# swapUniba/Deep_CBRS_Amar_Renaissance

Hardware: AMD Instinct MI355X
Metric: (user,item) pairs scored/sec, ML-1M basic-gnn 2-layer, 1/2/4/8 MI355X (higher is better)
Workload: dtype f32; 1 GPU; ml1m(s=64) user-item graph: N=590592 nodes, nnz(A_hat)=55909934, 12089292 test pairs; econfigs/basic-gnn.yaml grid1 BasicGCN d=8 L=2 concat, dense [24,24], clf [48,48]; one propagation + per-entity towers + all pairs (shuffled order) per step (hoisted); scale=64, parallelism=single GPU (step replayed from a hipGraph)

## Files before the change

deep_cbrs_amar_renaissance_amd/capi.py:

```python
import ctypes
import os

import torch

_HERE = os.path.dirname(os.path.abspath(__file__))
LIB_PATH = os.path.join(_HERE, 'libamar_hip.so')

ACT_NONE, ACT_RELU, ACT_SIGMOID = 0, 1, 2
ACT_CODES = {None: ACT_NONE, 'linear': ACT_NONE, 'relu': ACT_RELU, 'sigmoid': ACT_SIGMOID}
AGG_SUM, AGG_MAX, AGG_MIN = 0, 1, 2
AGG_CODES = {'sum': AGG_SUM, 'max': AGG_MAX, 'min': AGG_MIN}
SPMM_BIAS, SPMM_RELU, SPMM_ACCUM, SPMM_ACCUM_DIV, SPMM_SCALE_NEXT, SPMM_SAGE_TAIL, SPMM_LT_NOPAIRS = 1, 2, 4, 8, 16, 32, 64

_P = ctypes.c_void_p
_I32, _I64, _U32, _F32 = ctypes.c_int32, ctypes.c_int64, ctypes.c_uint32, ctypes.c_float

SIGNATURES = {
    'amar_version': (ctypes.c_int, []),
    'amar_error_string': (ctypes.c_char_p, [ctypes.c_int]),
    'amar_last_hip_error': (ctypes.c_int, []),
    'amar_spmm_csr_f32': (ctypes.c_int, [_P, _P, _P, _P, _I64, _P, _I64, _I32, _I32, _U32, _P,
                                         _P, _I64, _P, _I64, _F32, _P]),
    'amar_spmm_sj_f32': (ctypes.c_int, [_P, _P, _P, _I32, _P, _I64, _P, _I64, _I32, _I32, _U32, _P,
                                        _P, _I64, _P, _I64, _F32, _P, _I32, _P, _I64, _P]),
# ... 4 lines not shown
    'amar_gat_lt_rows_per_wave': (ctypes.c_int, [_I32]),
    'amar_colmax_f32': (ctypes.c_int, [_P, _I64, _P, _P]),
    'amar_spmm_lt_f32': (ctypes.c_int, [_P, _P, _P, _P, _P, _P, _P, _I32, _I32, _I32, _P, _P, _P, _I64, _I32, _P, _P, _I64, _I32, _I32, _U32, _P,
                                        _P, _I64, _P, _I64, _F32, _P, _I32, _P, _I64, _P]),
    'amar_propagate_route': (ctypes.c_int, [_I32, _I64, _I64, _I32, _U32, _P]),
    'amar_gat_xs_f32': (ctypes.c_int, [_P, _P, _I32, _P, _I64, _I32, _P, _P, _P, _P, _P, _P, _I64, _I32, _I32, _I32, _I32, _P]),
    'amar_gcn_layer_f32': (ctypes.c_int, [_P, _P, _P, _P, _I64, _I32, _P, _P, _I64, _P, _I32, _P, _I64, _I32, _P]),
    'amar_rowwise_xw_f32': (ctypes.c_int, [_P, _I64, _I32, _P, _I32, _P, _I64, _P, _I64, _P, _P, _P, _P, _P, _I32, _P]),
    'amar_rowwise_xw_gather_f32': (ctypes.c_int, [_P, _I64, _I32, _P, _P, _I32, _P, _I64, _P, _I32, _P]),
    'amar_sage_layer_f32': (ctypes.c_int, [_P, _P, _P, _I64, _I32, _P, _P, _I32, _P, _I64, _I32, _I32, _P]),
    'amar_sage_tail_f32': (ctypes.c_int, [_P, _I64, _P, _I64, _I32, _P, _P, _I32, _P, _I64, _I64, _P]),
    'amar_sage_layer_agg_f32': (ctypes.c_int, [_P, _P, _P, _I64, _I32, _P, _P, _I32, _P, _I64, _I32, _I32, _I32, _P]),
    'amar_sage_aggregate_f32': (ctypes.c_int, [_P, _P, _P, _I64, _I32, _P, _I64, _P, _I64, _I32, _I32, _I32, _P]),
    'amar_sage_aggregate_bwd_f32': (ctypes.c_int, [_P, _P, _P, _I64, _P, _I64, _P, _I64, _P, _I64, _I32, _P, _P, _I64, _I32, _I32, _P]),
    'amar_gat_layer_f32': (ctypes.c_int, [_P, _P, _P, _I64, _I32, _P, _P, _P, _P, _I64, _I32, _I32, _P]),
    'amar_rowwise_xw_heads_f32': (ctypes.c_int, [_P, _I64, _I32, _P, _I32, _I32, _P, _I64, _P, _P, _P, _I32, _P]),
    'amar_gat_heads_f32': (ctypes.c_int, [_P, _P, _P, _I64, _I32, _I32, _P, _P, _P, _I64, _P, _I32, _I32, _I32, _P]),
    'amar_dense_f32': (ctypes.c_int, [_P, _I64, _P, _P, _P, _P, _I64, _I64, _I32, _I32, _I32, _P]),
    'amar_dense_route': (ctypes.c_int, [_P, _I64, _P, _P, _P, _P, _I64, _I64, _I32, _I32, _I32, _P]),
    'amar_dense_split_bytes': (ctypes.c_int64, [_I32, _I32]),
    'amar_dense_split_pack_f32': (ctypes.c_int, [_P, _I32, _I32, _P]),
    'amar_dense_split_f32': (ctypes.c_int, [_P, _I64, _P, _P, _P, _P, _I64, _I64, _I32, _I32, _I32, _P]),
    'amar_chain_pack_floats': (ctypes.c_int64, [_P, _I32]),
    'amar_chain_pack_f32': (ctypes.c_int, [_P, _P, _P, _I32, _P]),
    'amar_chain_f32': (ctypes.c_int, [_P, _I64, _I32, _P, _I32, _P, _I64, _I32, _P, _I32, _I32, _I32, _P, _P, _P, _I32, _P, _I64, _I64, _P]),
    'amar_chain_indexed_f32': (ctypes.c_int, [_P, _I64, _I32, _P, _I32, _P, _I64, _I32, _P, _I32, _I32, _I32, _P, _P, _P, _I32, _P, _I64, _P, _I64, _P]),
    'amar_chain_segments_f32': (ctypes.c_int, [_P, _P, _P, _I32, _P, _I32, _P, _P, _P, _I32, _P, _I64, _I64, _P]),
    'amar_chain_route': (ctypes.c_int, [_P, _I64, _I32, _P, _I32, _P, _I64, _I32, _P, _I32, _I32, _I32, _P, _P, _P, _I32, _P, _I64, _P, _I64, _P]),
    'amar_chain_segments_route': (ctypes.c_int, [_P, _P, _P, _I32, _P, _I32, _P, _P, _P, _I32, _P, _I64, _I64, _P]),
    'amar_dual_chain_f32': (ctypes.c_int, [_P, _P, _P, _P, _P, _P, _P, _P, _I32, _I32, _I32, _P, _P, _P, _I32, _P, _P, _I64, _I64, _P]),
    'amar_dual_chain_indexed_f32': (ctypes.c_int, [_P, _P, _P, _P, _P, _P, _P, _P, _I32, _I32, _I32, _P, _P, _P, _I32, _P, _P, _I64, _P, _I64, _P]),
    'amar_copy_columns_f32': (ctypes.c_int, [_P, _I64, _P, _I32, _P, _I64, _I64, _I32, _P]),
    'amar_scatter_f32': (ctypes.c_int, [_P, _P, _P, _I64, _I64, _P, _I32, _P]),
    'amar_reduce_layers_f32': (ctypes.c_int, [_P, _I64, _I32, _I32, _P, _I64, _I64, _I32, _P]),
    'amar_reduce_layers_wsum_f32': (ctypes.c_int, [_P, _I64, _I32, _I32, _P, _P, _I64, _I64, _P]),
    'amar_reduce_layers_wsum_bwd_scratch': (ctypes.c_int64, []),
    'amar_reduce_layers_wsum_bwd_f32': (ctypes.c_int, [_P, _I64, _I32, _I32, _P, _P, _I64, _P, _I64, _P, _P, _I64, _P]),
    'amar_act_bwd_f32': (ctypes.c_int, [_P, _I64, _P, _I64, _P, _I64, _I64, _I32, _I32, _P]),
    'amar_wgrad_scratch_floats': (ctypes.c_int64, [_I64, _I32, _I32]),
    'amar_wgrad_f32': (ctypes.c_int, [_P, _I64, _P, _I64, _I64, _I32, _I32, _P, _P, _P, _P]),
    'amar_dense_stack_f32': (ctypes.c_int, [_P, _I64, _P, _P, _I64, _I32, _P, _P, _P, _P, _P, _P, _I64, _P]),
    'amar_dense_stack_pair_f32': (ctypes.c_int, [_P, _P, _P]),
    'amar_dense_stack_route': (ctypes.c_int, [_P, _I64, _P, _P, _I64, _I32, _P, _P, _P, _P, _P, _P, _I64, _P]),
    'amar_dense_stack_bwd_groups': (ctypes.c_int64, [_I64]),
    'amar_dense_stack_bwd_workspace_floats': (ctypes.c_int64, [_I64, _I32, _P]),
    'amar_dense_stack_bwd_pair_f32': (ctypes.c_int, [_P, _P, _P]),
    'amar_dense_stack_bwd_f32': (ctypes.c_int, [_P, _I64, _P, _I64, _I32, _P, _P, _P, _P, _P, _P, _I64, _P, _P, _P, _I32, _I64, _P]),
    'amar_dense_stack_bwd_route': (ctypes.c_int, [_P, _I64, _P, _I64, _I32, _P, _P, _P, _P, _P, _P, _I64, _P, _P, _P, _I32, _I64, _P]),
    'amar_dense_bwd_workspace_floats': (ctypes.c_int64, [_I64, _I32, _I32]),
    'amar_dense_bwd_groups': (ctypes.c_int64, [_I64]),
    'amar_dense_bwd_f32': (ctypes.c_int, [_P, _I64, _P, _I64, _P, _I64, _P, _I32, _P, _I64, _P, _P, _P, _I64, _P, _I64, _I32, _I32, _P]),
    'amar_dense_bwd_route': (ctypes.c_int, [_P, _I64, _P, _I64, _P, _I64, _P, _I32, _P, _I64, _P, _P, _P, _I64, _I64, _I32, _I32, _P]),
    'amar_bce_grad_f32': (ctypes.c_int, [_P, _I64, _P, _P, _P, _I64, _P]),
    'amar_wgrad_route': (ctypes.c_int, [_P, _I64, _P, _I64, _I64, _I32, _I32, _P, _P, _P]),
    'amar_scatter_add_rows_route': (ctypes.c_int, [_I64, _I32, _P]),
    'amar_scatter_add_rows_f32': (ctypes.c_int, [_P, _I64, _P, _I32, _P, _I64, _I64, _I32, _P]),
    'amar_add_inplace_f32': (ctypes.c_int, [_P, _I64, _P, _I64, _I64, _I32, _F32, _P]),
    'amar_row_affine_f32': (ctypes.c_int, [_P, _I64, _P, _I64, _P, _P, _I64, _I64, _I32, _P]),
    'amar_l2norm_fwd_f32': (ctypes.c_int, [_P, _I64, _P, _I64, _P, _P, _I64, _I64, _I32, _I32, _P]),
    'amar_l2norm_bwd_f32': (ctypes.c_int, [_P, _I64, _P, _I64, _P, _P, _I64, _I64, _I32, _I32, _P]),
    'amar_gat_bwd_f32': (ctypes.c_int, [_P, _P, _P, _I64, _I32, _P, _P, _P, _I64, _P, _I64, _P, _P, _P, _P, _P, _P, _P, _P, _I64,
                                        _I32, _I32, _P]),
    'amar_gat_bwd_directed_f32': (ctypes.c_int, [_P, _P, _P, _P, _P, _I64, _I32, _P, _P, _P, _I64, _P, _I64, _P, _P, _P, _P, _P, _P, _P, _P, _I64,
                                                 _I32, _I32, _P]),
    'amar_gat_heads_bwd_f32': (ctypes.c_int, [_P, _P, _P, _P, _P, _I64, _I32, _I32, _P, _P, _I64, _P, _I64, _P, _P, _P, _P, _P, _P, _P, _P, _I64,
                                              _I32, _I32, _I32, _P]),
# ... 797 lines not shown


def dual_chain_supported(D, n_branch_dims_equal, trunk_dims):
    return (D % 16 == 0 and D <= 64 and n_branch_dims_equal and len(trunk_dims) >= 3 and trunk_dims[0] == 2 * D
            and trunk_dims[-1] == 1 and len(set(trunk_dims[1:-1])) == 1 and trunk_dims[1] <= 64 and trunk_dims[1] % 4 == 0)


def dual_chain(tables_a, tables_b, ids_a, ids_b, bases_a, bases_b, D, in_act, branch_acts, trunk_dims, trunk_acts, wpack, out,
               out_index=None):
    P = out.shape[0]
    arr = lambda vals, ctype: (ctype * 2)(*vals)
    A = arr([_ptr(t, torch.float32, 'A') for t in tables_a], ctypes.c_void_p)
    B = arr([_ptr(t, torch.float32, 'B') for t in tables_b], ctypes.c_void_p)
    IA = arr([_ptr(t, torch.int32, 'ida') for t in ids_a], ctypes.c_void_p)
    IB = arr([_ptr(t, torch.int32, 'idb') for t in ids_b], ctypes.c_void_p)
    for ids in list(ids_a) + list(ids_b):
        if ids is not None and ids.numel() != P:
            raise ValueError("dual_chain: one id per output row expected")
    lda = arr([_ld(t, 'A') for t in tables_a], ctypes.c_int64)
    ldb = arr([_ld(t, 'B') for t in tables_b], ctypes.c_int64)
    ba, bb = arr([int(b) for b in bases_a], ctypes.c_int32), arr([int(b) for b in bases_b], ctypes.c_int32)
    bacts = (ctypes.c_int32 * max(1, len(branch_acts)))(*[ACT_CODES[a] for a in branch_acts])
    tdims = (ctypes.c_int32 * len(trunk_dims))(*trunk_dims)
    tacts = (ctypes.c_int32 * len(trunk_acts))(*[ACT_CODES[a] for a in trunk_acts])
    if out_index is not None and out_index.numel() != P:
        raise ValueError("dual_chain: out_index must have one entry per output row")
    code = load().amar_dual_chain_indexed_f32(A, lda, IA, ba, B, ldb, IB, bb, D, ACT_CODES[in_act], len(branch_acts), bacts,
                                              tdims, tacts, len(trunk_acts), _ptr(wpack, torch.float32, 'wpack'),
                                              _ptr(out, torch.float32, 'out'), _ld(out, 'out'), _ptr(out_index, torch.int32, 'out_index'),
                                              P, _stream())
    _check(code, 'amar_dual_chain_f32' if out_index is None else 'amar_dual_chain_indexed_f32')


def scatter(src, index, dst, window_off=None, n_windows=1):
    n = int(index.numel())
    if src.numel() < n or (window_off is not None and window_off.numel() != n_windows + 1):
        raise ValueError("scatter: one source value per index and n_windows + 1 window offsets expected")
    if n == 0:
        return
    _check(load().amar_scatter_f32(_ptr(src, torch.float32, 'src'), _ptr(index, torch.int32, 'index'), _ptr(dst, torch.float32, 'dst'),
                                   _ld(dst, 'dst') if dst.dim() == 2 else 1, n, _ptr(window_off, torch.int32, 'window_off'),
                                   int(n_windows), _stream()), 'amar_scatter_f32')


def copy_columns(src, dst, ids=None, base=0):
    n = ids.numel() if ids is not None else src.shape[0]
    if src.shape[1] != dst.shape[1] or dst.shape[0] != n:
        raise ValueError("copy_columns: shapes differ")
    code = load().amar_copy_columns_f32(_ptr(src, torch.float32, 'src'), _ld(src, 'src'),
                                        _ptr(ids, torch.int32, 'ids'), int(base),
                                        _ptr(dst, torch.float32, 'dst'), _ld(dst, 'dst'),
                                        n, src.shape[1], _stream())
    _check(code, 'amar_copy_columns_f32')


def reduce_layers(cat, n_layers, width, out, mean=False):
    if cat.shape[1] != n_layers * width or tuple(out.shape) != (cat.shape[0], width):
        raise ValueError("reduce_layers: cat [n, n_layers*width], out [n, width] expected")
    code = load().amar_reduce_layers_f32(_ptr(cat, torch.float32, 'cat'), _ld(cat, 'cat'), n_layers, width,
                                         _ptr(out, torch.float32, 'out'), _ld(out, 'out'), cat.shape[0],
                                         1 if mean else 0, _stream())
    _check(code, 'amar_reduce_layers_f32')


def reduce_layers_wsum(cat, n_layers, width, w, out):
    if cat.shape[1] != n_layers * width or tuple(out.shape) != (cat.shape[0], width) or w.numel() != n_layers or not w.is_contiguous():
        raise ValueError("reduce_layers_wsum: cat [n, n_layers*width], w [n_layers], out [n, width] expected")
    code = load().amar_reduce_layers_wsum_f32(_ptr(cat, torch.float32, 'cat'), _ld(cat, 'cat'), n_layers, width, _ptr(w, torch.float32, 'w'),
                                              _ptr(out, torch.float32, 'out'), _ld(out, 'out'), cat.shape[0], _stream())
    _check(code, 'amar_reduce_layers_wsum_f32')


def reduce_layers_wsum_bwd(cat, n_layers, width, w, d_out, d_cat, dw):
    n = cat.shape[0]
# ... 1055 lines not shown
```

deep_cbrs_amar_renaissance_amd/csrc/amar_layout.hip:

```cpp
#include "amar_common.h"

namespace {

__global__ __launch_bounds__(256) void copy_columns_kernel(const float *__restrict__ src, int64_t lds,
                                                           const int32_t *__restrict__ ids, int base,
                                                           float *__restrict__ dst, int64_t ldd, int64_t n_rows,
                                                           int width) {
    const int64_t total = n_rows * width;
    for (int64_t i = (int64_t)blockIdx.x * blockDim.x + threadIdx.x; i < total; i += (int64_t)gridDim.x * blockDim.x) {
        const int64_t r = i / width;
        const int c = (int)(i - r * width);
        const int64_t sr = ids ? (int64_t)ids[r] - base : r;
        dst[r * ldd + c] = src[sr * lds + c];
    }
}

__global__ __launch_bounds__(256) void copy_columns_vec_kernel(const float *__restrict__ src, int64_t lds,
                                                               const int32_t *__restrict__ ids, int base,
                                                               float *__restrict__ dst, int64_t ldd, int64_t n_rows,
                                                               int quads) {
    const int64_t total = n_rows * quads;
    for (int64_t i = (int64_t)blockIdx.x * blockDim.x + threadIdx.x; i < total; i += (int64_t)gridDim.x * blockDim.x) {
        const int64_t r = i / quads;
        const int q = (int)(i - r * quads);
// ... 46 lines not shown
#pragma unroll
        for (int l = 0; l < WSUM_MAX_LAYERS; ++l)
            if (l < n_layers) {
                acc[l] = fmaf(g, cat[r * ld + (int64_t)l * width + c], acc[l]);
                d_cat[r * ldc + (int64_t)l * width + c] = ww[l] * g;
            }
    }
#pragma unroll
    for (int l = 0; l < WSUM_MAX_LAYERS; ++l) {
        float v = acc[l];
        for (int off = 32; off > 0; off >>= 1) v += __shfl_xor(v, off, 64);
        if ((threadIdx.x & 63) == 0) red[threadIdx.x >> 6][l] = v;
    }
    __syncthreads();
    if (threadIdx.x < WSUM_MAX_LAYERS)
        partials[(int64_t)blockIdx.x * WSUM_MAX_LAYERS + threadIdx.x] =
            ((red[0][threadIdx.x] + red[1][threadIdx.x]) + red[2][threadIdx.x]) + red[3][threadIdx.x];
}

__global__ __launch_bounds__(64) void reduce_layers_wsum_dw_kernel(const float *__restrict__ partials, int n_blocks, int n_layers,
                                                                   const float *__restrict__ w, float *__restrict__ dw) {
    const int l = blockIdx.x;
    float v = 0.f;
    for (int b = threadIdx.x; b < n_blocks; b += 64) v += partials[(int64_t)b * WSUM_MAX_LAYERS + l];
    for (int off = 32; off > 0; off >>= 1) v += __shfl_xor(v, off, 64);
    if (threadIdx.x == 0 && l < n_layers) dw[l] = 2.f * w[l] * v;
}

unsigned grid_for(int64_t total) {
    int64_t b = (total + 255) / 256;
    return (unsigned)(b > 4096 ? 4096 : (b < 1 ? 1 : b));
}

__global__ __launch_bounds__(256) void scatter_windows_kernel(const float *__restrict__ src, const int32_t *__restrict__ index,
                                                              float *__restrict__ dst, int64_t ldd, int64_t n,
                                                              const int32_t *__restrict__ window_off, int n_windows, int per_xcd) {
    const int x = blockIdx.x & 7, j = blockIdx.x >> 3;
    for (int w = x; w < n_windows; w += 8) {
        const int64_t lo = window_off ? window_off[w] : n * w / n_windows, hi = window_off ? window_off[w + 1] : n * (w + 1) / n_windows;
        const int64_t step = (int64_t)per_xcd * 256;
        int64_t t = lo + (int64_t)j * 256 + threadIdx.x;
        for (; t + 3 * step < hi; t += 4 * step) {
            const int32_t i0 = index[t], i1 = index[t + step], i2 = index[t + 2 * step], i3 = index[t + 3 * step];
            const float v0 = src[t], v1 = src[t + step], v2 = src[t + 2 * step], v3 = src[t + 3 * step];
            dst[(int64_t)i0 * ldd] = v0; dst[(int64_t)i1 * ldd] = v1; dst[(int64_t)i2 * ldd] = v2; dst[(int64_t)i3 * ldd] = v3;
        }
        for (; t < hi; t += step) dst[(int64_t)index[t] * ldd] = src[t];
    }
}

}

extern "C" {

int amar_copy_columns_f32(const float *src, int64_t lds, const int32_t *ids, int32_t base,
                          float *dst, int64_t ldd, int64_t n_rows, int32_t width, amar_stream_t stream) {
    if (n_rows < 0 || width < 1 || !src || !dst || lds < width || ldd < width) return AMAR_EINVAL;
    if (n_rows == 0) return AMAR_OK;
    if ((width & 3) == 0 && (lds & 3) == 0 && (ldd & 3) == 0 && amar_aligned16(src) && amar_aligned16(dst))
        hipLaunchKernelGGL(copy_columns_vec_kernel, dim3(grid_for(n_rows * (width / 4))), dim3(256), 0,
                           static_cast<hipStream_t>(stream), src, lds, ids, base, dst, ldd, n_rows, width / 4);
    else
        hipLaunchKernelGGL(copy_columns_kernel, dim3(grid_for(n_rows * width)), dim3(256), 0,
                           static_cast<hipStream_t>(stream), src, lds, ids, base, dst, ldd, n_rows, width);
    return amar_check_launch();
}

int amar_reduce_layers_f32(const float *cat, int64_t ld, int32_t n_layers, int32_t width, float *out, int64_t ldo,
                           int64_t n_rows, int32_t mean, amar_stream_t stream) {
    if (n_rows < 0 || n_layers < 1 || width < 1 || !cat || !out || ld < (int64_t)n_layers * width || ldo < width)
// ... 10 lines not shown
    if (n_rows < 0 || n_layers < 1 || width < 1 || !cat || !w || !out || ld < (int64_t)n_layers * width || ldo < width)
        return AMAR_EINVAL;
    if (n_layers > WSUM_MAX_LAYERS) return AMAR_EUNSUPPORTED;
    if (n_rows == 0) return AMAR_OK;
    hipLaunchKernelGGL(reduce_layers_wsum_kernel, dim3(grid_for(n_rows * width)), dim3(256), 0,
                       static_cast<hipStream_t>(stream), cat, ld, n_layers, width, w, out, ldo, n_rows);
    return amar_check_launch();
}

int64_t amar_reduce_layers_wsum_bwd_scratch(void) { return (int64_t)WSUM_BWD_BLOCKS * WSUM_MAX_LAYERS; }

int amar_reduce_layers_wsum_bwd_f32(const float *cat, int64_t ld, int32_t n_layers, int32_t width, const float *w,
                                    const float *d_out, int64_t ldd, float *d_cat, int64_t ld_dcat, float *dw, float *scratch,
                                    int64_t n_rows, amar_stream_t stream) {
    if (n_rows < 0 || n_layers < 1 || width < 1 || !cat || !w || !d_out || !d_cat || !dw || !scratch ||
        ld < (int64_t)n_layers * width || ld_dcat < (int64_t)n_layers * width || ldd < width)
        return AMAR_EINVAL;
    if (n_layers > WSUM_MAX_LAYERS) return AMAR_EUNSUPPORTED;
    hipStream_t st = static_cast<hipStream_t>(stream);
    int64_t blocks = (n_rows * width + 255) / 256;
    if (blocks > WSUM_BWD_BLOCKS) blocks = WSUM_BWD_BLOCKS;
    if (blocks < 1) blocks = 1;
    hipLaunchKernelGGL(reduce_layers_wsum_bwd_kernel, dim3((unsigned)blocks), dim3(256), 0, st, cat, ld, n_layers, width, w, d_out, ldd,
                       d_cat, ld_dcat, n_rows, scratch);
    hipLaunchKernelGGL(reduce_layers_wsum_dw_kernel, dim3((unsigned)n_layers), dim3(64), 0, st, scratch, (int)blocks, n_layers, w, dw);
    return amar_check_launch();
}

int amar_scatter_f32(const float *src, const int32_t *index, float *dst, int64_t ldd, int64_t n, const int32_t *window_off,
                     int32_t n_windows, amar_stream_t stream) {
    if (n < 0 || !src || !index || !dst || ldd < 1 || n_windows < 1 || n >= (1ll << 31)) return AMAR_EINVAL;
    if (n == 0) return AMAR_OK;
    constexpr int per_xcd = 32;
    hipLaunchKernelGGL(scatter_windows_kernel, dim3(8 * per_xcd), dim3(256), 0, static_cast<hipStream_t>(stream), src, index, dst, ldd, n,
                       window_off, n_windows, per_xcd);
    return amar_check_launch();
}
}
```

deep_cbrs_amar_renaissance_amd/models/basic.py:

```python
import abc

import os

import numpy as np

import torch

from deep_cbrs_amar_renaissance_amd import capi
from deep_cbrs_amar_renaissance_amd import recommend as rec
from deep_cbrs_amar_renaissance_amd.engine import Model, ids_to_device, to_device_tensor
from deep_cbrs_amar_renaissance_amd.models.dense import build_dense_network, build_dense_classifier
from deep_cbrs_amar_renaissance_amd.models.gnn import GCN, GAT, GraphSage, LightGCN, DGCF
from deep_cbrs_amar_renaissance_amd.models.tsgnn import TwoStepGCN, TwoStepGraphSage, TwoStepGAT, TwoStepLightGCN, TwoStepDGCF
from deep_cbrs_amar_renaissance_amd.models.twgnn import TwoWayGCN, TwoWayGraphSage, TwoWayGAT, TwoWayLightGCN, TwoWayDGCF


class BasicRS(rec.SimilarSearch, Model):
    def __init__(
            self,
            dense_units=(512, 256, 128),
            clf_units=(64, 64),
            activation='relu',
            **kwargs
    ):
# ... 71 lines not shown

    def tower(self, key, table, ids=None):
        plan = self._split_plan(table.shape[1], table.shape[1])
        if plan is None:
            return (self.unet if key == 'u' else self.inet).apply2(table, ids_a=ids)
        blob, dims, acts = plan[key]
        m = ids.numel() if ids is not None else table.shape[0]
        t = torch.empty((m, dims[-1]), dtype=torch.float32, device=table.device)
        capi.chain(table, blob, dims, acts, t, ids_a=ids)
        return t

    def split_ready(self):
        return self._split_cache[1] is not None

    def score_towers(self, towers, u_ids, i_ids, u_base=0, i_base=0, pair_plan=None):
        tu, ti, split = towers
        if not split:
            return self.clf.apply2(tu, ti, ids_a=u_ids, base_a=u_base, ids_b=i_ids, base_b=i_base)
        plan = self._split_cache[1]
        blob, dims, acts = plan['rest']
        m = u_ids.numel() if u_ids is not None else tu.shape[0]
        out = torch.empty((m, 1), dtype=torch.float32, device=tu.device)
        if u_ids is None or i_ids is None:
            rows = getattr(self, '_row_ids', None)
            if rows is None or rows.numel() < m or rows.device != tu.device:
                rows = self._row_ids = torch.arange(max(m, 4096), dtype=torch.int32, device=tu.device)
            u_ids, u_base = (rows[:m], 0) if u_ids is None else (u_ids, u_base)
            i_ids, i_base = (rows[:m], 0) if i_ids is None else (i_ids, i_base)
        if pair_plan is not None:
            pair_plan.check(u_ids, i_ids)
            if pair_plan.mid_index is not None:
                capi.chain(tu, blob, dims, acts, pair_plan.mid.view(-1, 1), ids_a=pair_plan.u_ids, base_a=u_base, B=ti, ids_b=pair_plan.i_ids,
                           base_b=i_base, sum_inputs=True, in_act=plan['in_act'], out_index=pair_plan.mid_index)
                capi.scatter(pair_plan.mid, pair_plan.final_index, out, pair_plan.window_off, pair_plan.n_windows)
                return out
            capi.chain(tu, blob, dims, acts, out, ids_a=pair_plan.u_ids, base_a=u_base, B=ti, ids_b=pair_plan.i_ids, base_b=i_base,
                       sum_inputs=True, in_act=plan['in_act'], out_index=pair_plan.out_index)
            return out
        capi.chain(tu, blob, dims, acts, out, ids_a=u_ids, base_a=u_base, B=ti, ids_b=i_ids, base_b=i_base,
                   sum_inputs=True, in_act=plan['in_act'])
        return out

    def recommend(self, trainset, k=10, users=None, exclude_seen=True):
        rec.check_k(k)
        rec.check_users(users, len(trainset.users))
        tables = self._recommend_tables(trainset)
        split = self._recommend_split(*tables)
        if split is not None:
            return rec.fused(split, split[2], trainset, k, users, exclude_seen)
        return self._recommend_pairs(trainset, k, users, exclude_seen, towers=self.towers(*tables))

    def _recommend_pairs(self, trainset, k=10, users=None, exclude_seen=True, towers=None):
        rec.check_k(k)
        rec.check_users(users, len(trainset.users))
        towers = towers if towers is not None else self.towers(*self._recommend_tables(trainset))
        return rec.pairs(lambda u, i: self.score_towers(towers, u, i), trainset, k, users, exclude_seen, device=towers[0].device)

    def _recommend_route(self, trainset):
        d = np.asarray(trainset.embeddings).shape[1]
        if not self.built:
            self.build_head(d, d)
        return 'fused' if self._split_plan(d, d) is not None or self._rank_plan() is not None else 'pairs'

    def _recommend_tables(self, trainset):
        n_users, n_items = len(trainset.users), len(trainset.items)
        table = to_device_tensor(trainset.embeddings)
        if not self.built:
# ... 9 lines not shown

    def _rank_plan(self):
        clf = list(self.clf.layers)
        if len(clf) < 3 or clf[-1].units != 1 or len(clf) - 1 > capi.CHAIN_MAX_LAYERS + 1:
            return None
        rdims = [clf[0].units] + [l.units for l in clf[1:]]
        if max(rdims) > capi.CHAIN_MAX_WIDTH or rdims[0] % 4:
            return None
        np_ = lambda p: p.detach().cpu().numpy()
        rb, _ = capi.chain_pack([np_(l.kernel) for l in clf[1:]], [np_(l.bias) for l in clf[1:]])
        return {'rest': (torch.from_numpy(rb).to(clf[0].kernel.device), rdims, [l.activation for l in clf[1:]]), 'in_act': clf[0].activation}

    def _recommend_split(self, u_table, i_table):
        plan = self._split_plan(u_table.shape[1], i_table.shape[1])
        if plan is not None:
            tu, ti, _ = self.towers(u_table, i_table)
            return tu, ti, plan
        plan = self._rank_plan()
        if plan is None:
            return None
        tu_full, ti_full = self.unet.apply2(u_table), self.inet.apply2(i_table)
        l0 = self.clf.layers[0]
        w1, d, c1 = l0.kernel.detach(), tu_full.shape[1], l0.units
        tu = torch.empty((tu_full.shape[0], c1), dtype=torch.float32, device=tu_full.device)
        ti = torch.empty((ti_full.shape[0], c1), dtype=torch.float32, device=ti_full.device)
        capi.dense(tu_full, w1[:d].contiguous(), None, tu, act=None)
        capi.dense(ti_full, w1[d:].contiguous(), l0.bias.detach().contiguous(), ti, act=None)
        return tu, ti, plan

class PairPlan:

    N_XCD, CHUNK = 8, 128

    def __init__(self, u_ids, i_ids, phases=1):
        p = int(u_ids.numel())
        dev = u_ids.device
        pos = torch.arange(p, device=dev)
        per_phase = -(-p // phases)
        cls = (pos // per_phase) * self.N_XCD + (pos // self.CHUNK) % self.N_XCD
        n_cls = phases * self.N_XCD
        slots = torch.bincount(cls, minlength=n_cls)
        by_item = torch.argsort(i_ids.to(torch.int64), stable=True)
        order_cls = torch.arange(n_cls, device=dev).view(phases, self.N_XCD).t().reshape(-1)
        bucket_sizes = slots[order_cls]
        bucket_of_rank = torch.repeat_interleave(order_cls, bucket_sizes)
        order = by_item[torch.argsort((bucket_of_rank * (int(u_ids.max()) + 1) + u_ids[by_item].to(torch.int64)) * p + by_item)] if p else by_item
        place = torch.argsort(cls * p + pos)
        src = torch.empty(p, dtype=torch.int64, device=dev)
        src[place] = order
        self.u_ids = u_ids[src].contiguous()
        self.i_ids = i_ids[src].contiguous()
        self.out_index = src.to(torch.int32).contiguous()
        self._key = (u_ids.data_ptr(), i_ids.data_ptr(), p)
        self.window = 1 << max(16, min(19, int(round(np.log2(max(p, 1) / 185.0)))))
        self.mid_index = self.final_index = self.window_off = self.mid = None
        self.n_windows = 0
        if p > 2 * self.window and p >= int(os.environ.get('AMAR_PAIR_WINDOW_MIN', str(1 << 22))):
            n_win = -(-p // self.window)
            key = (src // self.window) * self.N_XCD + (pos // self.CHUNK) % self.N_XCD
            by_key = torch.argsort(key * p + pos)
            mid_index = torch.empty(p, dtype=torch.int32, device=dev)
            mid_index[by_key] = torch.arange(p, dtype=torch.int32, device=dev)
            self.mid_index = mid_index
            self.final_index = self.out_index[by_key].contiguous()
            counts = torch.bincount(src // self.window, minlength=n_win)
            self.window_off = torch.cat([torch.zeros(1, dtype=torch.int64, device=dev), torch.cumsum(counts, 0)]).to(torch.int32)
            self.n_windows = n_win
            self.mid = torch.empty(p, dtype=torch.float32, device=dev)

    def check(self, u_ids, i_ids):
        if (u_ids.data_ptr(), i_ids.data_ptr(), int(u_ids.numel())) != self._key:
            raise ValueError("this PairPlan was prepared for another pair list")


class BasicGNN(rec.SimilarSearch, Model, abc.ABC):
    def __init__(
            self,
            dense_units=(32, 16),
            clf_units=(16, 16),
            activation='relu',
            **kwargs
    ):
        super().__init__()
        self.rs = BasicRS(dense_units, clf_units, activation=activation)
        self.n_users = self.n_items = None
        self._towers = None
        self.built = True

    def call(self, inputs, **kwargs):
        updated_embeddings = self.gnn(None)
        return self.embed_recommend(updated_embeddings, inputs)

    def embed_recommend(self, embeddings, inputs):
        n_nodes = embeddings.shape[0]
        u, i = ids_to_device(inputs[0], n_nodes), ids_to_device(inputs[1], n_nodes)
        if not self.gnn.hoist:
            return self.rs([embeddings, embeddings], u_ids=u, i_ids=i)
        key = (self.weights_version, embeddings.data_ptr())
        if self._towers is None or self._towers[0] != key:
            n = embeddings.shape[0]
            nu = self.n_users if self.n_users is not None else n
# ... 101 lines not shown
```

deep_cbrs_amar_renaissance_amd/models/hybrid.py:

```python
import abc
import os

import numpy as np
import torch

from deep_cbrs_amar_renaissance_amd import capi
from deep_cbrs_amar_renaissance_amd import recommend as rec
from deep_cbrs_amar_renaissance_amd.engine import Model, ids_to_device, to_device_tensor
from deep_cbrs_amar_renaissance_amd.layers.fusion import FusionLayer
from deep_cbrs_amar_renaissance_amd.models.dense import build_dense_classifier, build_dense_network, build_residual_dense_network
from deep_cbrs_amar_renaissance_amd.models.gnn import GCN, GAT, GraphSage, LightGCN, DGCF
from deep_cbrs_amar_renaissance_amd.models.tsgnn import TwoStepGCN, TwoStepGraphSage, TwoStepGAT, TwoStepLightGCN, TwoStepDGCF
from deep_cbrs_amar_renaissance_amd.models.twgnn import TwoWayGCN, TwoWayGraphSage, TwoWayGAT, TwoWayLightGCN, TwoWayDGCF


class HybridCBRS(rec.SimilarSearch, Model):

    def __init__(
            self,
            feature_based=True,
            dense_units=((512, 256, 128), (512, 256, 128), (64, 64)),
            clf_units=(64, 64),
            activation='relu',
            fusion_method='concatenate',
# ... 155 lines not shown
            args2 = args1
            in1, in2 = (tug, tig), (tub, tib)
        else:
            args1 = dict(ids_a=u_ids, base_a=u_base, ids_b=u_ids, base_b=u_base)
            args2 = dict(ids_a=i_ids, base_a=i_base, ids_b=i_ids, base_b=i_base)
            in1, in2 = (tug, tub), (tig, tib)
        plain = self.fuse2.method == 'concatenate' and self.residual is None
        if not folded:
            if self.fuse1a.method == 'concatenate':
                x1 = self.dense3a.apply2(in1[0], in1[1], **args1)
                x2 = self.dense3b.apply2(in2[0], in2[1], **args2)
            else:
                xs = []
                for fuse, net, (ta, tb), args in ((self.fuse1a, self.dense3a, in1, args1), (self.fuse1b, self.dense3b, in2, args2)):
                    ga, gb = self._rows(ta, args['ids_a'], args['base_a']), self._rows(tb, args['ids_b'], args['base_b'])
                    xs.append(net.apply2(fuse([ga, gb])))
                x1, x2 = xs
            return self.clf.apply2(x1, x2) if plain else self._tail(x1, x2)
        plan = self._dual_plan() if plain else None
        if plan is not None:
            m = args1['ids_a'].numel() if args1['ids_a'] is not None else in1[0].shape[0]
            out = torch.empty((m, 1), dtype=torch.float32, device=in1[0].device)
            if pair_plan is not None and u_ids is not None and i_ids is not None:
                pair_plan.check(u_ids, i_ids)
                pu, pi = pair_plan.u_ids, pair_plan.i_ids
                ia, ib = ((pu, pu), (pi, pi)) if self.feature_based else ((pu, pi), (pu, pi))
                two_step = pair_plan.mid_index is not None
                capi.dual_chain((in1[0], in2[0]), (in1[1], in2[1]), ia, ib,
                                (args1['base_a'], args2['base_a']), (args1['base_b'], args2['base_b']),
                                plan['D'], plan['in_act'], plan['branch_acts'], plan['trunk_dims'], plan['trunk_acts'], plan['wpack'],
                                pair_plan.mid.view(-1, 1) if two_step else out,
                                out_index=pair_plan.mid_index if two_step else pair_plan.out_index)
                if two_step:
                    capi.scatter(pair_plan.mid, pair_plan.final_index, out, pair_plan.window_off, pair_plan.n_windows)
                return out
            capi.dual_chain((in1[0], in2[0]), (in1[1], in2[1]), (args1['ids_a'], args2['ids_a']), (args1['ids_b'], args2['ids_b']),
                            (args1['base_a'], args2['base_a']), (args1['base_b'], args2['base_b']),
                            plan['D'], plan['in_act'], plan['branch_acts'], plan['trunk_dims'], plan['trunk_acts'], plan['wpack'], out)
            return out
        outs = []
        for net, (ta, tb), args in ((self.dense3a, in1, args1), (self.dense3b, in2, args2)):
            blob, dims, acts, in_act = self._rest(net)
            m = args['ids_a'].numel() if args['ids_a'] is not None else ta.shape[0]
            x = torch.empty((m, dims[-1]), dtype=torch.float32, device=ta.device)
            capi.chain(ta, blob, dims, acts, x, B=tb, sum_inputs=True, in_act=in_act, **args)
            outs.append(x)
        return self.clf.apply2(outs[0], outs[1]) if plain else self._tail(outs[0], outs[1])

    def recommend(self, trainset, k=10, users=None, exclude_seen=True):
        return self._recommend_pairs(trainset, k, users, exclude_seen)

    def _recommend_pairs(self, trainset, k=10, users=None, exclude_seen=True, towers=None):
        rec.check_k(k)
        rec.check_users(users, len(trainset.users))
        towers = towers if towers is not None else self._recommend_towers(trainset)
        return rec.pairs(lambda u, i: self.score_towers(towers, u, i), trainset, k, users, exclude_seen, device=towers[0].device)

    def _recommend_route(self, trainset):
        return 'pairs'

    def _recommend_towers(self, trainset):
        n_users, n_items = len(trainset.users), len(trainset.items)
        g, b = to_device_tensor(trainset.graph_embeddings), to_device_tensor(trainset.bert_embeddings)
        if not self.built:
            self.build_head(g.shape[1], b.shape[1])
        return self.towers(g[:n_users], g[n_users:n_users + n_items], b[:n_users], b[n_users:n_users + n_items])

# ... 214 lines not shown
```

include/amar_hip.h:

```cpp
#ifndef AMAR_HIP_H
#define AMAR_HIP_H

#include <stdint.h>

#ifdef __cplusplus
extern "C" {
#endif

#define AMAR_OK            0
#define AMAR_EINVAL       -1
#define AMAR_EUNSUPPORTED -2
#define AMAR_ELAUNCH      -3

#define AMAR_ACT_NONE     0
#define AMAR_ACT_RELU     1
#define AMAR_ACT_SIGMOID  2
#define AMAR_DENSE_WT 0x100

#define AMAR_SPMM_BIAS      1u
#define AMAR_SPMM_RELU      2u
#define AMAR_SPMM_ACCUM     4u
#define AMAR_SPMM_ACCUM_DIV 8u
#define AMAR_SPMM_SCALE_NEXT 16u
#define AMAR_SPMM_SAGE_TAIL 32u
// ... 152 lines not shown
typedef struct amar_chain_route_info {
    int32_t kernel, maxt, full, am, split, scatter, shape, lastlin, seg, has_dot, layers, threads;
    int64_t blocks, lds_bytes;
} amar_chain_route_info;
int amar_chain_route(const float *A, int64_t lda, int32_t Da, const int32_t *ids_a, int32_t base_a,
                     const float *B, int64_t ldb, int32_t Db, const int32_t *ids_b, int32_t base_b,
                     int32_t sum_inputs, int32_t in_act,
                     const float *wpack, const int32_t *dims, const int32_t *acts, int32_t n_layers,
                     float *out, int64_t ldo, const int32_t *out_index, int64_t P, amar_chain_route_info *info);
int amar_chain_segments_route(const float *const *seg, const int64_t *seg_ld, const int32_t *seg_width, int32_t n_seg,
                              const int32_t *ids, int32_t base,
                              const float *wpack, const int32_t *dims, const int32_t *acts, int32_t n_layers,
                              float *out, int64_t ldo, int64_t P, amar_chain_route_info *info);

int amar_dual_chain_f32(const float *const *A, const int64_t *lda, const int32_t *const *ida, const int32_t *base_a,
                        const float *const *B, const int64_t *ldb, const int32_t *const *idb, const int32_t *base_b,
                        int32_t D, int32_t in_act, int32_t n_branch, const int32_t *branch_acts,
                        const int32_t *trunk_dims, const int32_t *trunk_acts, int32_t n_trunk,
                        const float *wpack, float *out, int64_t ldo, int64_t P, amar_stream_t stream);
int amar_dual_chain_indexed_f32(const float *const *A, const int64_t *lda, const int32_t *const *ida, const int32_t *base_a,
                                const float *const *B, const int64_t *ldb, const int32_t *const *idb, const int32_t *base_b,
                                int32_t D, int32_t in_act, int32_t n_branch, const int32_t *branch_acts,
                                const int32_t *trunk_dims, const int32_t *trunk_acts, int32_t n_trunk,
                                const float *wpack, float *out, int64_t ldo, const int32_t *out_index, int64_t P,
                                amar_stream_t stream);

int amar_copy_columns_f32(const float *src, int64_t lds, const int32_t *ids, int32_t base,
                          float *dst, int64_t ldd, int64_t n_rows, int32_t width, amar_stream_t stream);
int amar_reduce_layers_f32(const float *cat, int64_t ld, int32_t n_layers, int32_t width, float *out, int64_t ldo,
                           int64_t n_rows, int32_t mean, amar_stream_t stream);

int amar_scatter_f32(const float *src, const int32_t *index, float *dst, int64_t ldd, int64_t n,
                     const int32_t *window_off, int32_t n_windows, amar_stream_t stream);

int amar_reduce_layers_wsum_f32(const float *cat, int64_t ld, int32_t n_layers, int32_t width, const float *w, float *out, int64_t ldo,
                                int64_t n_rows, amar_stream_t stream);
int64_t amar_reduce_layers_wsum_bwd_scratch(void);
int amar_reduce_layers_wsum_bwd_f32(const float *cat, int64_t ld, int32_t n_layers, int32_t width, const float *w,
                                    const float *d_out, int64_t ldd, float *d_cat, int64_t ld_dcat, float *dw, float *scratch,
                                    int64_t n_rows, amar_stream_t stream);

int amar_gat_xs_f32(const int32_t *rowptr, const int32_t *colidx, int32_t n_slices,
                    const float *H, int64_t ldh, int32_t C, const float *s_self, const float *s_neigh, const float *bias,
                    float *packed, float *partials, float *Y, int64_t ldy, int32_t self_loop, int32_t n_rows,
                    int32_t n_cols, int32_t row_offset, amar_stream_t stream);

int amar_gat_lt_f32(const int32_t *words, const int32_t *stream_start, const int32_t *wsteps, const int32_t *tile_row0,
                    const int32_t *n_win, const int32_t *vstart, const int32_t *vcount, int32_t n_tiles, int32_t maxwin1, int32_t pace_every,
                    int32_t rows_per_wave, const float *diag, const int32_t *rowptr, const int32_t *colidx,
                    const float *H, int64_t ldh, int32_t C, const float *s_self, const float *s_neigh, const float *s_neigh_max,
                    const float *bias, float *Y, int64_t ldy, int32_t self_loop, int32_t n_rows, int32_t n_cols, int32_t row_offset,
                    amar_stream_t stream);
int amar_gat_lt_rows_per_wave(int32_t C);
int amar_colmax_f32(const float *x, int64_t n, float *out, amar_stream_t stream);

int amar_attention_mix_f32(const float *A, int64_t lda, const float *B, int64_t ldb, const float *TA, int64_t ldta,
                           const float *TB, int64_t ldtb, float *out, int64_t ldo, int64_t M, int32_t D, amar_stream_t stream);
int amar_attention_mix_bwd_f32(const float *dOut, int64_t ldd, const float *A, int64_t lda, const float *B, int64_t ldb,
                               const float *TA, int64_t ldta, const float *TB, int64_t ldtb,
                               float *dA, float *dB, float *dTA, float *dTB, int64_t M, int32_t D, amar_stream_t stream);
int amar_add3_act_f32(const float *A, int64_t lda, const float *B, int64_t ldb, const float *C, int64_t ldc, float *out, int64_t ldo,
                      int64_t M, int32_t W, int32_t act, amar_stream_t stream);
int amar_locality_scale_f32(const float *X, int64_t ldx, const float *w, float *out, int64_t ldo, int64_t M, int32_t W,
                            amar_stream_t stream);
int amar_locality_scale_bwd_f32(const float *dOut, int64_t ldd, const float *X, int64_t ldx, const float *w, float *dX, int64_t lddx,
                                float *dw, int64_t M, int32_t W, int32_t accumulate, amar_stream_t stream);
// ... 244 lines not shown
```

Measured before the change: 12.03 billion pairs/s.

## Scatter pair scores through LDS per closed window, sized to one window per CU

```diff
diff --git a/deep_cbrs_amar_renaissance_amd/capi.py b/deep_cbrs_amar_renaissance_amd/capi.py
--- a/deep_cbrs_amar_renaissance_amd/capi.py
+++ b/deep_cbrs_amar_renaissance_amd/capi.py
@@ -60,6 +60,7 @@
     'amar_dual_chain_indexed_f32': (ctypes.c_int, [_P, _P, _P, _P, _P, _P, _P, _P, _I32, _I32, _I32, _P, _P, _P, _I32, _P, _P, _I64, _P, _I64, _P]),
     'amar_copy_columns_f32': (ctypes.c_int, [_P, _I64, _P, _I32, _P, _I64, _I64, _I32, _P]),
     'amar_scatter_f32': (ctypes.c_int, [_P, _P, _P, _I64, _I64, _P, _I32, _P]),
+    'amar_scatter_closed_f32': (ctypes.c_int, [_P, _P, _P, _I64, _P, _I32, _I32, _P]),
     'amar_reduce_layers_f32': (ctypes.c_int, [_P, _I64, _I32, _I32, _P, _I64, _I64, _I32, _P]),
     'amar_reduce_layers_wsum_f32': (ctypes.c_int, [_P, _I64, _I32, _I32, _P, _P, _I64, _I64, _P]),
     'amar_reduce_layers_wsum_bwd_scratch': (ctypes.c_int64, []),
@@ -923,14 +924,31 @@
     _check(code, 'amar_dual_chain_f32' if out_index is None else 'amar_dual_chain_indexed_f32')
 
 
-def scatter(src, index, dst, window_off=None, n_windows=1):
+SCATTER_CLOSED_MAX_WINDOW = 65536
+
+
+def scatter_route(n, ldd, max_window, closed):
+    if os.environ.get('AMAR_PAIR_SCATTER', '') == 'global':
+        return 'global'
+    if not closed or int(ldd) != 1 or int(n) <= 0 or max_window is None or not 1 <= int(max_window) <= SCATTER_CLOSED_MAX_WINDOW:
+        return 'global'
+    return 'lds'
+
+
+def scatter(src, index, dst, window_off=None, n_windows=1, closed=False, max_window=None):
     n = int(index.numel())
     if src.numel() < n or (window_off is not None and window_off.numel() != n_windows + 1):
         raise ValueError("scatter: one source value per index and n_windows + 1 window offsets expected")
     if n == 0:
         return
+    ldd = _ld(dst, 'dst') if dst.dim() == 2 else 1
+    if window_off is not None and scatter_route(n, ldd, max_window, closed) == 'lds':
+        _check(load().amar_scatter_closed_f32(_ptr(src, torch.float32, 'src'), _ptr(index, torch.int32, 'index'), _ptr(dst, torch.float32, 'dst'),
+                                              n, _ptr(window_off, torch.int32, 'window_off'), int(n_windows), int(max_window), _stream()),
+               'amar_scatter_closed_f32')
+        return
     _check(load().amar_scatter_f32(_ptr(src, torch.float32, 'src'), _ptr(index, torch.int32, 'index'), _ptr(dst, torch.float32, 'dst'),
-                                   _ld(dst, 'dst') if dst.dim() == 2 else 1, n, _ptr(window_off, torch.int32, 'window_off'),
+                                   ldd, n, _ptr(window_off, torch.int32, 'window_off'),
                                    int(n_windows), _stream()), 'amar_scatter_f32')
 
 
diff --git a/deep_cbrs_amar_renaissance_amd/csrc/amar_layout.hip b/deep_cbrs_amar_renaissance_amd/csrc/amar_layout.hip
--- a/deep_cbrs_amar_renaissance_amd/csrc/amar_layout.hip
+++ b/deep_cbrs_amar_renaissance_amd/csrc/amar_layout.hip
@@ -102,10 +102,61 @@
     return (unsigned)(b > 4096 ? 4096 : (b < 1 ? 1 : b));
 }
 
-__global__ __launch_bounds__(256) void scatter_windows_kernel(const float *__restrict__ src, const int32_t *__restrict__ index,
-                                                              float *__restrict__ dst, int64_t ldd, int64_t n,
-                                                              const int32_t *__restrict__ window_off, int n_windows, int per_xcd) {
+constexpr int SCATTER_CLOSED_THREADS = 1024;
+constexpr int SCATTER_CLOSED_PIECE = 32768;
+
+template <bool CLOSED>
+__global__ __launch_bounds__(CLOSED ? SCATTER_CLOSED_THREADS : 256) void scatter_windows_kernel(
+    const float *__restrict__ src, const int32_t *__restrict__ index, float *__restrict__ dst, int64_t ldd, int64_t n,
+    const int32_t *__restrict__ window_off, int n_windows, int per_xcd, int cap) {
     const int x = blockIdx.x & 7, j = blockIdx.x >> 3;
+    if constexpr (CLOSED) {
+        extern __shared__ float piece[];
+        const int parts = per_xcd, w = (j / parts) * 8 + x, part = j % parts;
+        if (w >= n_windows) return;
+        const int nn = (int)n;
+        const int lo = min(max(window_off[w], 0), nn), hi = min(max(window_off[w + 1], lo), nn), len = hi - lo;
+        const int plen = (len + parts - 1) / parts, dlo = lo + part * plen;
+        const int dn = min(min(plen, hi - dlo), cap);
+        if (dn <= 0) return;
+        const int a = (int)((reinterpret_cast<uintptr_t>(dst + dlo) >> 2) & 3);
+        const int tid = threadIdx.x, T = blockDim.x;
+        auto keep = [&](int32_t i, float v) {
+            const unsigned k = (unsigned)(i - dlo);
+            if (k < (unsigned)dn) piece[a + k] = v;
+        };
+        const int mis = (int)((reinterpret_cast<uintptr_t>(index + lo) >> 2) & 3);
+        const bool alike = mis == (int)((reinterpret_cast<uintptr_t>(src + lo) >> 2) & 3);
+        const int head = alike ? min(len, (4 - mis) & 3) : len, nq = (len - head) >> 2;
+        const int4 *iq = reinterpret_cast<const int4 *>(index + lo + head);
+        const float4 *vq = reinterpret_cast<const float4 *>(src + lo + head);
+        int q = tid;
+        for (; q + 3 * T < nq; q += 4 * T) {
+            const int4 i0 = iq[q], i1 = iq[q + T], i2 = iq[q + 2 * T], i3 = iq[q + 3 * T];
+            const float4 v0 = vq[q], v1 = vq[q + T], v2 = vq[q + 2 * T], v3 = vq[q + 3 * T];
+            keep(i0.x, v0.x); keep(i0.y, v0.y); keep(i0.z, v0.z); keep(i0.w, v0.w);
+            keep(i1.x, v1.x); keep(i1.y, v1.y); keep(i1.z, v1.z); keep(i1.w, v1.w);
+            keep(i2.x, v2.x); keep(i2.y, v2.y); keep(i2.z, v2.z); keep(i2.w, v2.w);
+            keep(i3.x, v3.x); keep(i3.y, v3.y); keep(i3.z, v3.z); keep(i3.w, v3.w);
+        }
+        for (; q < nq; q += T) {
+            const int4 i0 = iq[q];
+            const float4 v0 = vq[q];
+            keep(i0.x, v0.x); keep(i0.y, v0.y); keep(i0.z, v0.z); keep(i0.w, v0.w);
+        }
+        for (int t = tid; t < head; t += T) keep(index[lo + t], src[lo + t]);
+        for (int t = head + 4 * nq + tid; t < len; t += T) keep(index[lo + t], src[lo + t]);
+        __syncthreads();
+        float *d = dst + dlo - a;
+        const int end = a + dn, vs = min((a + 3) & ~3, end), ve = max(end & ~3, vs);
+        for (int s = vs + 4 * tid; s < ve; s += 4 * T)
+            *reinterpret_cast<float4 *>(d + s) = *reinterpret_cast<const float4 *>(piece + s);
+        if (tid < 4) {
+            if (a + tid < vs) d[a + tid] = piece[a + tid];
+            if (ve + tid < end) d[ve + tid] = piece[ve + tid];
+        }
+        return;
+    }
     for (int w = x; w < n_windows; w += 8) {
         const int64_t lo = window_off ? window_off[w] : n * w / n_windows, hi = window_off ? window_off[w + 1] : n * (w + 1) / n_windows;
         const int64_t step = (int64_t)per_xcd * 256;
@@ -182,8 +233,28 @@
     if (n < 0 || !src || !index || !dst || ldd < 1 || n_windows < 1 || n >= (1ll << 31)) return AMAR_EINVAL;
     if (n == 0) return AMAR_OK;
     constexpr int per_xcd = 32;
-    hipLaunchKernelGGL(scatter_windows_kernel, dim3(8 * per_xcd), dim3(256), 0, static_cast<hipStream_t>(stream), src, index, dst, ldd, n,
-                       window_off, n_windows, per_xcd);
-    return amar_check_launch();
-}
-}
+    hipLaunchKernelGGL(scatter_windows_kernel<false>, dim3(8 * per_xcd), dim3(256), 0, static_cast<hipStream_t>(stream), src, index, dst, ldd, n,
+                       window_off, n_windows, per_xcd, 0);
+    return amar_check_launch();
+}
+
+int amar_scatter_closed_f32(const float *src, const int32_t *index, float *dst, int64_t n, const int32_t *window_off, int32_t n_windows,
+                            int32_t max_window, amar_stream_t stream) {
+    static_assert(AMAR_SCATTER_CLOSED_MAX_WINDOW % SCATTER_CLOSED_PIECE == 0, "a window of the capacity is cut into whole pieces");
+    if (n < 0 || !src || !index || !dst || !window_off || n_windows < 1 || n >= (1ll << 31) || max_window < 0 ||
+        max_window > AMAR_SCATTER_CLOSED_MAX_WINDOW || (int64_t)max_window * n_windows < n)
+        return AMAR_EINVAL;
+    if (n == 0) return AMAR_OK;
+    const int parts = (max_window + SCATTER_CLOSED_PIECE - 1) / SCATTER_CLOSED_PIECE;
+    const int cap = (max_window + parts - 1) / parts;
+    const size_t lds = (size_t)(cap + 4) * sizeof(float);
+    auto kern = scatter_windows_kernel<true>;
+    static bool allowed[AMAR_MAX_DEVICES] = {};
+    if (const int rc = amar_allow_lds(reinterpret_cast<const void *>(kern), (SCATTER_CLOSED_PIECE + 4) * sizeof(float), allowed)) return rc;
+    const int64_t groups = ((int64_t)n_windows + 7) / 8 * 8 * parts;
+    if (groups >= (1ll << 31)) return AMAR_EINVAL;
+    hipLaunchKernelGGL(kern, dim3((unsigned)groups), dim3(SCATTER_CLOSED_THREADS), lds, static_cast<hipStream_t>(stream), src, index, dst, (int64_t)1, n,
+                       window_off, n_windows, parts, cap);
+    return amar_check_launch();
+}
+}
diff --git a/deep_cbrs_amar_renaissance_amd/models/basic.py b/deep_cbrs_amar_renaissance_amd/models/basic.py
--- a/deep_cbrs_amar_renaissance_amd/models/basic.py
+++ b/deep_cbrs_amar_renaissance_amd/models/basic.py
@@ -127,7 +127,8 @@
             if pair_plan.mid_index is not None:
                 capi.chain(tu, blob, dims, acts, pair_plan.mid.view(-1, 1), ids_a=pair_plan.u_ids, base_a=u_base, B=ti, ids_b=pair_plan.i_ids,
                            base_b=i_base, sum_inputs=True, in_act=plan['in_act'], out_index=pair_plan.mid_index)
-                capi.scatter(pair_plan.mid, pair_plan.final_index, out, pair_plan.window_off, pair_plan.n_windows)
+                capi.scatter(pair_plan.mid, pair_plan.final_index, out, pair_plan.window_off, pair_plan.n_windows, closed=True,
+                             max_window=pair_plan.max_window)
                 return out
             capi.chain(tu, blob, dims, acts, out, ids_a=pair_plan.u_ids, base_a=u_base, B=ti, ids_b=pair_plan.i_ids, base_b=i_base,
                        sum_inputs=True, in_act=plan['in_act'], out_index=pair_plan.out_index)
@@ -203,7 +204,7 @@
 
     N_XCD, CHUNK = 8, 128
 
-    def __init__(self, u_ids, i_ids, phases=1):
+    def __init__(self, u_ids, i_ids, phases=1, window=None):
         p = int(u_ids.numel())
         dev = u_ids.device
         pos = torch.arange(p, device=dev)
@@ -223,9 +224,9 @@
         self.i_ids = i_ids[src].contiguous()
         self.out_index = src.to(torch.int32).contiguous()
         self._key = (u_ids.data_ptr(), i_ids.data_ptr(), p)
-        self.window = 1 << max(16, min(19, int(round(np.log2(max(p, 1) / 185.0)))))
+        self.window = int(window) if window else self.window_for(p)
         self.mid_index = self.final_index = self.window_off = self.mid = None
-        self.n_windows = 0
+        self.n_windows = self.max_window = 0
         if p > 2 * self.window and p >= int(os.environ.get('AMAR_PAIR_WINDOW_MIN', str(1 << 22))):
             n_win = -(-p // self.window)
             key = (src // self.window) * self.N_XCD + (pos // self.CHUNK) % self.N_XCD
@@ -235,9 +236,17 @@
             self.mid_index = mid_index
             self.final_index = self.out_index[by_key].contiguous()
             counts = torch.bincount(src // self.window, minlength=n_win)
+            self.max_window = int(counts.max())
             self.window_off = torch.cat([torch.zeros(1, dtype=torch.int64, device=dev), torch.cumsum(counts, 0)]).to(torch.int32)
             self.n_windows = n_win
             self.mid = torch.empty(p, dtype=torch.float32, device=dev)
+
+    @classmethod
+    def window_for(cls, p):
+        by_cu = -(-(-(-max(p, 1) // 256)) // cls.CHUNK) * cls.CHUNK
+        if capi.scatter_route(p, 1, by_cu, True) == 'lds':
+            return by_cu
+        return 1 << max(16, min(19, int(round(np.log2(max(p, 1) / 185.0)))))
 
     def check(self, u_ids, i_ids):
         if (u_ids.data_ptr(), i_ids.data_ptr(), int(u_ids.numel())) != self._key:
diff --git a/deep_cbrs_amar_renaissance_amd/models/hybrid.py b/deep_cbrs_amar_renaissance_amd/models/hybrid.py
--- a/deep_cbrs_amar_renaissance_amd/models/hybrid.py
+++ b/deep_cbrs_amar_renaissance_amd/models/hybrid.py
@@ -211,7 +211,8 @@
                                 pair_plan.mid.view(-1, 1) if two_step else out,
                                 out_index=pair_plan.mid_index if two_step else pair_plan.out_index)
                 if two_step:
-                    capi.scatter(pair_plan.mid, pair_plan.final_index, out, pair_plan.window_off, pair_plan.n_windows)
+                    capi.scatter(pair_plan.mid, pair_plan.final_index, out, pair_plan.window_off, pair_plan.n_windows, closed=True,
+                                 max_window=pair_plan.max_window)
                 return out
             capi.dual_chain((in1[0], in2[0]), (in1[1], in2[1]), (args1['ids_a'], args2['ids_a']), (args1['ids_b'], args2['ids_b']),
                             (args1['base_a'], args2['base_a']), (args1['base_b'], args2['base_b']),
diff --git a/include/amar_hip.h b/include/amar_hip.h
--- a/include/amar_hip.h
+++ b/include/amar_hip.h
@@ -208,6 +208,10 @@
 
 int amar_scatter_f32(const float *src, const int32_t *index, float *dst, int64_t ldd, int64_t n,
                      const int32_t *window_off, int32_t n_windows, amar_stream_t stream);
+
+#define AMAR_SCATTER_CLOSED_MAX_WINDOW 65536
+int amar_scatter_closed_f32(const float *src, const int32_t *index, float *dst, int64_t n, const int32_t *window_off,
+                            int32_t n_windows, int32_t max_window, amar_stream_t stream);
 
 int amar_reduce_layers_wsum_f32(const float *cat, int64_t ld, int32_t n_layers, int32_t width, const float *w, float *out, int64_t ldo,
                                 int64_t n_rows, amar_stream_t stream);
```

New measurement: 12.40 billion pairs/s (median of 6 runs). 1.03x the previous value.
